# senikm/trpx

Hardware: AMD Instinct MI355X
Metric: frames/s (Terse encode + Prolix decode round trip, 512x512 uint16 stack, bit-exact vs CPU ref) (higher is better)
Workload: dtype u16

## Files before the change

trpx_amd/csrc/encode_fused.hip:

```cpp
#include <stddef.h>
#include <utility>
#include "codec_common.hpp"
#include "launchers.hpp"
#include "profile.hpp"
#include <stdlib.h>
#include <mutex>
#include <vector>

namespace trpx {

#ifndef TRPX_FUSED_SUB32
#define TRPX_FUSED_SUB32 5
#endif
#ifndef TRPX_FUSED_SUB16
#define TRPX_FUSED_SUB16 4
#endif
template <typename T> constexpr int sub_tiles() { return sizeof(T) <= 2 ? TRPX_FUSED_SUB16 : TRPX_FUSED_SUB32; }
#ifndef TRPX_FUSED_OCC16
#define TRPX_FUSED_OCC16 8
#endif
#ifndef TRPX_FUSED_OCC32
#define TRPX_FUSED_OCC32 4
#endif
template <typename T> constexpr int fused_occupancy() { return sizeof(T) == 1 ? 8 : (sizeof(T) == 2 ? TRPX_FUSED_OCC16 : TRPX_FUSED_OCC32); }
[[maybe_unused]] constexpr uint64_t kWaitTicks = 25u * 1000u * 1000u;
struct SpinGuard {
    uint64_t t0 = 0;
    uint32_t spins = 0;
    __device__ __forceinline__ bool expired() {
#ifdef TRPX_FORCE_TIMEOUT
        return true;
#else
        if ((++spins & 63u) != 0u) return false;
        const uint64_t now = __builtin_amdgcn_s_memrealtime();
        if (t0 == 0) { t0 = now; return false; }
        return now - t0 > kWaitTicks;
#endif
    }
};

#ifdef TRPX_DIAGNOSTICS
#define TRPX_DIAG(a) ((a).debug)
#else
#define TRPX_DIAG(a) 0u
#endif

constexpr uint64_t kStInvalid = 0, kStAgg = 1, kStPrefix = 2;
constexpr uint32_t kGridY = 32768;
constexpr int kWmaxShift = 56;
constexpr uint64_t kBndHead = 1ull << 55;
constexpr uint64_t kHeadFlag = 1ull << 63, kTailFlag = 1ull << 62;
__device__ __forceinline__ uint64_t make_desc(uint64_t st, uint64_t v) { return (st << 62) | (v & ((1ull << 62) - 1)); }
__device__ __forceinline__ uint64_t desc_status(uint64_t d) { return d >> 62; }
__device__ __forceinline__ uint64_t desc_value(uint64_t d) { return d & ((1ull << 62) - 1); }

__device__ __forceinline__ uint64_t ld_desc(const uint64_t* p) {
    return __hip_atomic_load(p, __ATOMIC_RELAXED, __HIP_MEMORY_SCOPE_AGENT);
}
__device__ __forceinline__ void st_desc(uint64_t* p, uint64_t v) {
    __hip_atomic_store(p, v, __ATOMIC_RELAXED, __HIP_MEMORY_SCOPE_AGENT);
}

__device__ __forceinline__ uint64_t wave_sum64(uint64_t v) {
    const uint32_t l0 = (uint32_t)v & 0x1FFFFFu, l1 = (uint32_t)(v >> 21) & 0x1FFFFFu, l2 = (uint32_t)(v >> 42);
    const uint32_t s0 = (uint32_t)__builtin_amdgcn_readlane((int)wave_inclusive_scan(l0), 63);
    const uint32_t s1 = (uint32_t)__builtin_amdgcn_readlane((int)wave_inclusive_scan(l1), 63);
    const uint32_t s2 = (uint32_t)__builtin_amdgcn_readlane((int)wave_inclusive_scan(l2), 63);
    return (uint64_t)s0 + ((uint64_t)s1 << 21) + ((uint64_t)s2 << 42);
}

__device__ bool lookback(const uint64_t* __restrict__ desc, int64_t idx, int64_t lo, uint64_t* result) {
    const int lane = lane_id();
    uint64_t acc = 0;
    int64_t pos = idx - 1;
    while (pos >= lo) {
        const int64_t my = pos - lane;
        const bool in = my >= lo;
        uint64_t g = in ? 0ull : make_desc(kStPrefix, 0);
        uint32_t first_p = 64;
        SpinGuard guard;
        uint64_t need = ~0ull;
        for (;;) {
            if (desc_status(g) == kStInvalid && ((need >> lane) & 1ull)) g = ld_desc(desc + my);
            const uint64_t pmask = __ballot(desc_status(g) == kStPrefix);
            const uint64_t imask = __ballot(desc_status(g) == kStInvalid);
            first_p = pmask ? (uint32_t)__builtin_ctzll(pmask) : 64u;
            need = first_p >= 63u ? ~0ull : ((2ull << first_p) - 1ull);
            if ((imask & need) == 0) break;
            if (guard.expired()) return false;
            __builtin_amdgcn_s_sleep(2);
        }
        acc += wave_sum64((uint32_t)lane <= first_p ? desc_value(g) : 0ull);
        if (first_p < 64u) break;
        pos -= 64;
    }
    *result = acc;
    return true;
}

constexpr int kAccShift = 40;
#ifndef TRPX_FUSED_ACC_LINES
#define TRPX_FUSED_ACC_LINES 2
#endif
constexpr uint32_t kAccLines = TRPX_FUSED_ACC_LINES;
__host__ __device__ inline uint32_t fused_acc_lines(uint32_t tiles_per_frame) {
    const uint32_t k = (tiles_per_frame + 31u) / 32u;
    return k < 1u ? 1u : (k > kAccLines ? kAccLines : k);
}
constexpr uint64_t kPrefFlag = 1ull << 63;
__device__ bool lookback_frames(const uint64_t* __restrict__ acc_w, const uint64_t* __restrict__ pref_w, int64_t frame,
                                uint64_t tiles_per_frame, uint64_t* result, uint64_t stride, uint32_t n_acc) {
    const int lane = lane_id();
    uint64_t acc = 0;
    int64_t pos = frame - 1;
    while (pos >= 0) {
        const int64_t my = pos - lane;
        const bool in = my >= 0;
        uint64_t p = in ? 0ull : kPrefFlag, c = 0;
        uint32_t first_p = 64;
        SpinGuard guard;
        uint64_t need = ~0ull;
        bool complete = false;
        for (;;) {
            if (in && !(p & kPrefFlag) && !complete && ((need >> lane) & 1ull)) {
                p = ld_desc(pref_w + my * stride);
                c = ld_desc(acc_w + my * stride);
                for (uint32_t k = 1; k < n_acc; ++k) c += ld_desc(acc_w + my * stride + 16u * k);
                complete = (c >> kAccShift) == tiles_per_frame;
            }
            const uint64_t pmask = __ballot((p & kPrefFlag) != 0);
            const uint64_t cmask = __ballot(complete);
            first_p = pmask ? (uint32_t)__builtin_ctzll(pmask) : 64u;
            need = first_p >= 64u ? ~0ull : ((1ull << first_p) - 1ull);
            if ((~cmask & need) == 0) break;
            if (guard.expired()) return false;
            __builtin_amdgcn_s_sleep(2);
        }
        const uint64_t mine = (uint32_t)lane < first_p ? 1 + (c & ((1ull << kAccShift) - 1)) / 8
                                                       : ((uint32_t)lane == first_p ? p & ~kPrefFlag : 0ull);
        acc += wave_sum64(mine);
        if (first_p < 64u) break;
        pos -= 64;
    }
    *result = acc;
    return true;
}

template <typename T> struct Raw {
    static constexpr int bits = PixelTraits<T>::bits;
    static constexpr int per = 32 / bits;
    static constexpr int dw = kBlock / per;
};

template <typename T>
__device__ __forceinline__ uint32_t raw_field(const uint32_t (&raw)[Raw<T>::dw], int k) {
    constexpr int per = Raw<T>::per, bits = Raw<T>::bits;
    const uint32_t x = raw[k / per] >> ((k % per) * bits);
    return bits == 32 ? x : x & ((1u << (bits & 31)) - 1u);
}

template <typename T> struct QuadVec;
template <> struct QuadVec<uint8_t>  { typedef uint32_t type; };
template <> struct QuadVec<int8_t>   { typedef uint32_t type; };
template <> struct QuadVec<uint16_t> { typedef uint32_t type __attribute__((ext_vector_type(2))); };
template <> struct QuadVec<int16_t>  { typedef uint32_t type __attribute__((ext_vector_type(2))); };
template <> struct QuadVec<uint32_t> { typedef uint32_t type __attribute__((ext_vector_type(4))); };
template <> struct QuadVec<int32_t>  { typedef uint32_t type __attribute__((ext_vector_type(4))); };

template <typename T>
__device__ __forceinline__ void load_raw_nt(const T* __restrict__ p, uint32_t (&raw)[Raw<T>::dw]) {
    if constexpr (sizeof(T) == 2) {
        typedef uint32_t u4 __attribute__((ext_vector_type(4)));
        typedef uint32_t u2 __attribute__((ext_vector_type(2)));
        u4 lo; u2 hi;
        __builtin_memcpy(&lo, p, 16);
        __builtin_memcpy(&hi, reinterpret_cast<const char*>(p) + 16, 8);
        raw[0] = lo.x; raw[1] = lo.y; raw[2] = lo.z; raw[3] = lo.w; raw[4] = hi.x; raw[5] = hi.y;
        return;
    } else if constexpr (sizeof(T) == 1) {
        typedef uint32_t u3 __attribute__((ext_vector_type(3)));
        u3 x;
        __builtin_memcpy(&x, p, 12);
        raw[0] = x.x; raw[1] = x.y; raw[2] = x.z;
        return;
    }
    using V = typename QuadVec<T>::type;
    constexpr int q = Raw<T>::dw / 3;
    const V* src = reinterpret_cast<const V*>(p);
    union U { V vec; uint32_t x[q]; };
    U a, b, c;
    a.vec = src[0];
    b.vec = src[1];
    c.vec = src[2];
#pragma unroll
    for (int i = 0; i < q; ++i) { raw[i] = a.x[i]; raw[q + i] = b.x[i]; raw[2 * q + i] = c.x[i]; }
}
template <typename T>
__device__ __forceinline__ void load_raw_mis2(const T* __restrict__ p, uint32_t (&raw)[Raw<T>::dw]) {
    static_assert(sizeof(T) == 2, "16-bit pixels");
    typedef uint32_t u4 __attribute__((ext_vector_type(4)));
    typedef uint32_t u2 __attribute__((ext_vector_type(2)));
    const char* q = reinterpret_cast<const char*>(p) - 2;
    u4 lo; u2 hi; uint16_t last;
    __builtin_memcpy(&lo, q, 16);
    __builtin_memcpy(&hi, q + 16, 8);
    __builtin_memcpy(&last, q + 24, 2);
    raw[0] = __builtin_amdgcn_alignbit(lo.y, lo.x, 16); raw[1] = __builtin_amdgcn_alignbit(lo.z, lo.y, 16);
    raw[2] = __builtin_amdgcn_alignbit(lo.w, lo.z, 16); raw[3] = __builtin_amdgcn_alignbit(hi.x, lo.w, 16);
    raw[4] = __builtin_amdgcn_alignbit(hi.y, hi.x, 16); raw[5] = __builtin_amdgcn_alignbit((uint32_t)last, hi.y, 16);
}
template <typename T>
__device__ __forceinline__ void load_raw_partial(const T* __restrict__ p, int nb, uint32_t (&raw)[Raw<T>::dw]) {
    using UT = typename PixelTraits<T>::U;
#pragma unroll
    for (int i = 0; i < Raw<T>::dw; ++i) raw[i] = 0;
#pragma unroll
    for (int k = 0; k < kBlock; ++k)
        if (k < nb) raw[k / Raw<T>::per] |= (uint32_t)(UT)p[k] << ((k % Raw<T>::per) * Raw<T>::bits);
}

template <typename T>
__device__ __forceinline__ uint32_t raw_width(const uint32_t (&raw)[Raw<T>::dw]) {
    constexpr int bits = Raw<T>::bits;
    uint32_t m = 0;
    if (!PixelTraits<T>::is_signed) {
#pragma unroll
        for (int i = 0; i < Raw<T>::dw; ++i) m |= raw[i];
        if (bits == 16) m = (m | (m >> 16)) & 0xFFFFu;
        if (bits == 8) { m |= m >> 16; m = (m | (m >> 8)) & 0xFFu; }
    } else if (bits == 32) {
#pragma unroll
        for (int i = 0; i < Raw<T>::dw; ++i) {
            const uint32_t u = raw[i];
            m |= (int32_t)u < 0 ? 0u - u : u;
        }
    } else if (bits == 16) {
        typedef short s2 __attribute__((ext_vector_type(2)));
        typedef unsigned short us2 __attribute__((ext_vector_type(2)));
        uint32_t acc = 0;
#pragma unroll
        for (int i = 0; i < Raw<T>::dw; ++i) {
            union { uint32_t u; s2 v; us2 w; } x, n, y;
            x.u = raw[i];
            n.w = (us2)(0) - x.w;
            y.v = __builtin_elementwise_max(x.v, n.v);
            acc |= y.u;
        }
        m = (acc | (acc >> 16)) & 0xFFFFu;
    } else {
#pragma unroll
        for (int k = 0; k < kBlock; ++k) {
            const int32_t x = (int32_t)(int8_t)(raw[k / 4] >> ((k % 4) * 8));
            m |= (uint32_t)(x < 0 ? -x : x);
        }
    }
    return width_from_or<T>(m);
}

template <int ND>
__device__ __forceinline__ void lds_or_string(uint32_t* __restrict__ stage, uint32_t pos, uint32_t hv_top,
                                              const uint32_t* __restrict__ p) {
    const uint32_t d = (pos + 31u) >> 5, rs = (0u - pos) & 31u;
    const uint32_t xm = __builtin_amdgcn_alignbit(hv_top, 0u, rs);
    if (xm) atomicOr(&stage[d - 1], xm);
    if constexpr (ND == 0) {
        const uint32_t x0 = __builtin_amdgcn_alignbit(0u, hv_top, rs);
        if (x0) atomicOr(&stage[d], x0);
    } else {
        atomicOr(&stage[d], __builtin_amdgcn_alignbit(p[0], hv_top, rs));
#pragma unroll
        for (int j = 1; j < ND; ++j) {
            const uint32_t x = __builtin_amdgcn_alignbit(p[j], p[j - 1], rs);
            if (j >= ND - 1) atomicOr(&stage[d + j], x);
            else stage[d + j] = x;
        }
        const uint32_t x = __builtin_amdgcn_alignbit(0u, p[ND - 1], rs);
        if (x) atomicOr(&stage[d + ND], x);
    }
}

template <typename T, int W>
__device__ __forceinline__ void pack_payload_w(uint32_t* __restrict__ stage, uint32_t pos, uint32_t hv_top,
                                               const uint32_t (&raw)[Raw<T>::dw]) {
    constexpr int NB = kBlock * W;
    constexpr int ND = (NB + 31) / 32;
    constexpr int per = Raw<T>::per, bits = Raw<T>::bits;
    constexpr uint32_t MASK = W >= 32 ? 0xFFFFFFFFu : ((1u << (W & 31)) - 1u);
    uint32_t p[ND ? ND : 1];
#pragma unroll
    for (int j = 0; j < ND; ++j) p[j] = 0;
    if constexpr (W == 0) {
    } else if constexpr (bits == 16 && W < 16) {
        typedef unsigned short us2 __attribute__((ext_vector_type(2)));
        constexpr int L = (15 - W) / (2 * W) + 1;
        constexpr uint32_t kPairMask = MASK | (MASK << 16);
#pragma unroll
        for (int c = 0; c * L < kBlock / 2; ++c) {
            uint32_t acc = 0;
            int n_pairs = 0;
#pragma unroll
            for (int i = 0; i < L; ++i) {
                const int j = c * L + i;
                if (j < kBlock / 2) {
                    union { uint32_t u; us2 v; } x, k;
                    x.u = PixelTraits<T>::is_signed ? raw[j] & kPairMask : raw[j];
                    k.u = (1u << (2 * W * i)) | (1u << (2 * W * i + W + 16));
                    acc = __builtin_amdgcn_udot2(x.v, k.v, acc, false);
                    ++n_pairs;
                }
            }
            const int bit = 2 * W * L * c, nbits = 2 * W * n_pairs;
            p[bit >> 5] |= acc << (bit & 31);
            if ((bit & 31) + nbits > 32) p[(bit >> 5) + 1] |= acc >> (32 - (bit & 31));
        }
    } else if constexpr (bits == 16) {
#pragma unroll
        for (int j = 0; j < kBlock / 2; ++j) p[j] = raw[j];
    } else {
#pragma unroll
        for (int k = 0; k < kBlock; ++k) {
            const uint32_t u = (raw[k / per] >> ((k % per) * bits)) & MASK;
            const int bit = k * W;
            p[bit >> 5] |= u << (bit & 31);
            if ((bit & 31) + W > 32) p[(bit >> 5) + 1] |= u >> (32 - (bit & 31));
        }
    }
    lds_or_string<ND>(stage, pos, hv_top, p);
}

template <typename T, int LO, int HI>
struct PackDispatch {
    static __device__ __forceinline__ void run(uint32_t* stage, uint32_t pos, uint32_t hv_top, uint32_t w0,
                                               const uint32_t (&raw)[Raw<T>::dw]) {
        if constexpr (LO == HI) pack_payload_w<T, LO>(stage, pos, hv_top, raw);
        else {
            constexpr int MID = (LO + HI) / 2;
            if (w0 <= (uint32_t)MID) PackDispatch<T, LO, MID>::run(stage, pos, hv_top, w0, raw);
            else PackDispatch<T, MID + 1, HI>::run(stage, pos, hv_top, w0, raw);
        }
    }
};

template <typename T>
__device__ __forceinline__ void pack_payload_generic(uint32_t* __restrict__ stage, uint32_t pos, uint32_t w, int nb,
                                                     const uint32_t (&raw)[Raw<T>::dw]) {
    const uint32_t mask = w >= 32u ? 0xFFFFFFFFu : ((1u << w) - 1u);
#pragma unroll
    for (int k = 0; k < kBlock; ++k) {
        if (k < nb) {
            const uint64_t x = (uint64_t)(raw_field<T>(raw, k) & mask) << (pos & 31u);
            if ((uint32_t)x) atomicOr(&stage[pos >> 5], (uint32_t)x);
            if ((uint32_t)(x >> 32)) atomicOr(&stage[(pos >> 5) + 1], (uint32_t)(x >> 32));
            pos += w;
        }
    }
}

template <typename T> constexpr int fused_phase_rounds() { return (sub_tiles<T>() + 1) / 2; }
template <typename T>
constexpr int fused_stage_dwords() { return fused_phase_rounds<T>() * ((kThreads * max_block_bits<T>() + 31) / 32) + 12; }

struct FusedArgs {
    FrameGeom g;
    uint32_t n_frames;
    uint32_t tiles_per_frame;
    uint64_t out_capacity;
    uint64_t* tile_desc;
    uint64_t* tail_desc;
    uint64_t* bnd_pos;
    uint64_t* frame_acc;
    uint64_t* frame_pref;
    uint64_t* frame_base;
    uint32_t acc_stride;
    uint32_t n_acc;
    uint64_t* ws_tag;
    uint64_t expect_tag;
    uint64_t* frame_offsets;
    uint32_t* out32;
    uint32_t* status;
    uint8_t* idx_widths;
    uint64_t* idx_group_off;
    uint32_t debug;
    uint64_t* stamps;
};

typedef const char __attribute__((address_space(4)))* karg_ptr;
#define TRPX_KARG(kb, field) (*reinterpret_cast<const decltype(FusedArgs::field) __attribute__((address_space(4)))*>((kb) + 8 + offsetof(FusedArgs, field)))

template <typename T, bool MIS2>
__device__ __forceinline__ void encode_fused_body(const T* __restrict__ pixels, const FusedArgs& a) {
    constexpr int kSub = sub_tiles<T>();
    constexpr int kFusedTileBlocks = kSub * kThreads;
    constexpr int kStage = fused_stage_dwords<T>();
    constexpr int kStage4 = (kStage + 1 + 3) / 4;
    __shared__ __attribute__((aligned(16))) uint32_t s_stage_pad[4 * kStage4];
    uint32_t* const s_stage = s_stage_pad + 1;
    __shared__ uint32_t s_hdr[40];
    __shared__ uint32_t s_wtot[kSub * 4];
    __shared__ uint32_t s_wfl[kSub * 4];
    __shared__ uint64_t s_excl_bits;
    __shared__ uint64_t s_base_bytes;
    __shared__ uint32_t s_abort;
    __shared__ uint32_t s_carry;
    __shared__ uint32_t s_halo;

    const uint32_t tid = threadIdx.x;
#define TRPX_STAMP(slot) do { if ((TRPX_DIAG(a) & 4u) && threadIdx.x == 0) a.stamps[((uint64_t)(blockIdx.z * kGridY + blockIdx.y) * gridDim.x + blockIdx.x) * 8 + (slot)] = __builtin_amdgcn_s_memrealtime(); } while (0)
    TRPX_STAMP(0);
    const int lane = lane_id(), wave = wave_id();
    const FrameGeom g = a.g;
    const uint32_t t = blockIdx.x;
    const uint32_t frame = blockIdx.z * kGridY + blockIdx.y;
    const uint32_t n_frames = a.n_frames, tpf = a.tiles_per_frame;
    asm volatile("" :: "s"(g.n_values), "s"(g.n_blocks), "s"(n_frames), "s"(tpf), "s"(pixels));
    if (frame >= n_frames) return;
    const uint64_t tile = (uint64_t)frame * tpf + t;
    const bool last_tile_of_frame = t + 1 == tpf;
    if (tile == 0 && tid == 0) {
        karg_ptr kb0 = (karg_ptr)__builtin_amdgcn_kernarg_segment_ptr();
        uint64_t* const st64 = reinterpret_cast<uint64_t*>(TRPX_KARG(kb0, status));
#pragma unroll
        for (int i = 0; i < 4; ++i) st_desc(st64 + i, 0ull);
        const uint64_t want = TRPX_KARG(kb0, expect_tag);
        if (want != 0ull && ld_desc(TRPX_KARG(kb0, ws_tag)) != want) atomicMax(&TRPX_KARG(kb0, status)[0], 7u);
        asm volatile("s_waitcnt vmcnt(0)" ::: "memory");
    }
    const T* fp = pixels + (uint64_t)frame * g.n_values;
    const uint32_t b0 = t * kFusedTileBlocks;

    uint32_t v[kSub][Raw<T>::dw];
    uint32_t w[kSub], up[kSub], len[kSub], inc[kSub];
    int nb[kSub];
    const bool has_full = g.n_values >= (uint64_t)kBlock;
    const uint64_t max_first = has_full ? g.n_values - kBlock : 0;
    uint32_t h[Raw<T>::dw];
    [[maybe_unused]] const bool mis2 = MIS2 && ((uintptr_t)fp & 2u) != 0u && frame != 0u;
    if (has_full) {
        bool loaded = false;
        if constexpr (MIS2 && sizeof(T) == 2) {
            if (mis2) {
#pragma unroll
                for (int r = 0; r < kSub; ++r) {
                    const uint64_t first = (uint64_t)(b0 + r * kThreads + tid) * kBlock;
                    load_raw_mis2<T>(fp + (first < max_first ? first : max_first), v[r]);
                }
                loaded = true;
            }
        }
        if (!loaded) {
#pragma unroll
            for (int r = 0; r < kSub; ++r) {
                const uint64_t first = (uint64_t)(b0 + r * kThreads + tid) * kBlock;
                load_raw_nt<T>(fp + (first < max_first ? first : max_first), v[r]);
            }
        }
        if (wave == 0) load_raw_nt<T>(fp + (uint64_t)(b0 ? b0 - 1 : 0) * kBlock, h);
        else {
#pragma unroll
            for (int i = 0; i < Raw<T>::dw; ++i) h[i] = 0u;
        }
    } else {
#pragma unroll
        for (int r = 0; r < kSub; ++r)
#pragma unroll
            for (int i = 0; i < Raw<T>::dw; ++i) v[r][i] = 0u;
#pragma unroll
        for (int i = 0; i < Raw<T>::dw; ++i) h[i] = 0u;
    }
    const uint32_t nb_tail = (uint32_t)(g.n_values - (uint64_t)(g.n_blocks - 1) * kBlock);
#pragma unroll
    for (int r = 0; r < kSub; ++r) {
        const uint32_t b1 = b0 + r * kThreads + tid + 1u;
        nb[r] = b1 < g.n_blocks ? kBlock : (b1 == g.n_blocks ? (int)nb_tail : 0);
    }
    if (tid == 0) s_abort = 0;
    if (tid <= 32u) s_hdr[tid] = header_val(tid, tid + 1u) << (32u - header_len(tid, tid + 1u));
    {
        typedef uint32_t u4 __attribute__((ext_vector_type(4)));
        u4* z = reinterpret_cast<u4*>(s_stage_pad);
#pragma unroll
        for (int i = 0; i < (kStage4 + kThreads - 1) / kThreads; ++i)
            if (i * kThreads + (int)tid < kStage4) z[i * kThreads + tid] = (u4)(0u);
    }
    uint32_t pv[Raw<T>::dw];
#pragma unroll
    for (int i = 0; i < Raw<T>::dw; ++i) pv[i] = 0u;
    if (last_tile_of_frame && g.n_values % kBlock) {
        const uint32_t bp = g.n_blocks - 1;
        if (bp >= b0 && (bp - b0) % kThreads == tid) load_raw_partial<T>(fp + (uint64_t)bp * kBlock, (int)(g.n_values % kBlock), pv);
    }
    TRPX_STAMP(7);
    uint32_t w_part = 0u;
    if (last_tile_of_frame && g.n_values % kBlock) w_part = raw_width<T>(pv);
    if (wave == 0) {
        const uint32_t hw0 = b0 > 0 ? raw_width<T>(h) : 0u;
        if (lane == 0) s_halo = hw0;
    }
    uint32_t wmax = 0;
    uint32_t hlr[kSub];
#pragma unroll
    for (int r = 0; r < kSub; ++r) {
        w[r] = nb[r] == kBlock ? raw_width<T>(v[r]) : (nb[r] ? w_part : 0u);
        wmax = w[r] > wmax ? w[r] : wmax;
        if (a.idx_widths && nb[r]) a.idx_widths[(uint64_t)frame * g.n_blocks + b0 + r * kThreads + tid] = (uint8_t)w[r];
        up[r] = (uint32_t)__builtin_amdgcn_update_dpp(0, (int)w[r], 0x138, 0xf, 0xf, false);
        hlr[r] = header_len(w[r], up[r]);
        len[r] = nb[r] ? (lane ? hlr[r] : 0u) + (uint32_t)nb[r] * w[r] : 0u;
    }
    static_assert(kWave * max_block_bits<T>() < 65536, "packed scan needs 16-bit wave totals");
#pragma unroll
    for (int r = 0; r + 1 < kSub; r += 2) {
        const uint32_t two = wave_inclusive_scan(len[r] | (len[r + 1] << 16));
        inc[r] = two & 0xFFFFu;
        inc[r + 1] = two >> 16;
    }
    if (kSub & 1) inc[kSub - 1] = wave_inclusive_scan(len[kSub - 1]);
    const uint32_t wmax_wave = wave_max(wmax);
#pragma unroll
    for (int r = 0; r < kSub; ++r) {
        const uint32_t w_first = (uint32_t)__builtin_amdgcn_readfirstlane((int)w[r]);
        const uint32_t v_first = (uint32_t)__builtin_amdgcn_readfirstlane(nb[r]);
        if (lane == 63) {
            s_wtot[r * 4 + wave] = inc[r];
            s_wfl[r * 4 + wave] = w_first | (w[r] << 8) | ((v_first ? 1u : 0u) << 16) | (r == 0 ? wmax_wave << 24 : 0u);
        }
    }
    TRPX_STAMP(5);
    __syncthreads();
    TRPX_STAMP(1);

    const uint32_t tile_halo = s_halo;
    uint32_t rb[kSub + 1];
    uint32_t off[kSub];
    uint32_t meta[kSub];
    {
        uint32_t tot = 0, h0 = 0, wprev = 0;
        if (lane < kSub * 4) {
            const uint32_t wfl = s_wfl[lane];
            wprev = lane == 0 ? tile_halo : (s_wfl[lane - 1] >> 8) & 0xFFu;
            h0 = (wfl >> 16) & 1u ? header_len(wfl & 0xFFu, wprev) : 0u;
            tot = s_wtot[lane] + h0;
        }
        const uint32_t incl = wave_inclusive_scan(tot);
        const uint32_t excl = incl - tot;
        const uint32_t hw = h0 | (wprev << 8);
        const int swave = __builtin_amdgcn_readfirstlane(wave);
#pragma unroll
        for (int r = 0; r < kSub; ++r) {
            rb[r] = (uint32_t)__builtin_amdgcn_readlane((int)excl, r * 4);
            const uint32_t pb = (uint32_t)__builtin_amdgcn_readlane((int)excl, r * 4 + swave);
            const uint32_t ph = (uint32_t)__builtin_amdgcn_readlane((int)hw, r * 4 + swave);
            off[r] = pb + (lane ? (ph & 0xFFu) : 0u) + inc[r] - len[r];
            const uint32_t wp_r = lane ? up[r] : ph >> 8;
            const uint32_t hl_r = lane ? hlr[r] : (ph & 0xFFu);
            meta[r] = w[r] | (wp_r << 8) | (hl_r << 16) | (nb[r] == kBlock ? 1u << 24 : 0u) | (nb[r] ? 1u << 25 : 0u);
        }
        rb[kSub] = (uint32_t)__builtin_amdgcn_readlane((int)incl, kSub * 4 - 1);
    }
    const uint32_t tile_total = rb[kSub];

    if (tid == 0 && !(TRPX_DIAG(a) & 1u)) {
        st_desc(a.tile_desc + tile, make_desc(t == 0 ? kStPrefix : kStAgg, tile_total));
        __hip_atomic_fetch_add(a.frame_acc + (uint64_t)frame * a.acc_stride + 16u * (t % a.n_acc), (1ull << kAccShift) | tile_total, __ATOMIC_RELAXED, __HIP_MEMORY_SCOPE_AGENT);
    }
    constexpr int kPhaseRounds = fused_phase_rounds<T>();
    constexpr uint32_t kCapBits = (uint32_t)kPhaseRounds * kThreads * max_block_bits<T>();
    const bool two_phase = tile_total > kCapBits;
    uint64_t p0 = 0, p_end = 0;
    uint64_t img_p0 = 0;
    uint32_t bias = 0;
    bool writable = false;
#ifndef TRPX_ABLATE
#define TRPX_ABLATE 0
#endif
#define TRPX_WSTAMP(slot) do { if ((TRPX_DIAG(a) & 8u) && lane == 0 && tile < 4096) a.stamps[tile * 32 + wave * 8 + (slot)] = __builtin_amdgcn_s_memrealtime(); } while (0)
    auto pack_round = [&](auto rc) {
        constexpr int r = decltype(rc)::value;
        const uint32_t pos = off[r] - bias;
        const uint32_t mr = meta[r];
        const uint32_t hl = (mr >> 16) & 0xFFu;
        const uint32_t wr = mr & 0xFFu;
        const uint32_t hv_top = wr == ((mr >> 8) & 0xFFu) ? 0x80000000u : s_hdr[wr];
        const bool full = (mr >> 24) & 1u;
        if (((mr >> 25) & 1u) && !full && !(TRPX_ABLATE & 2)) {
            const uint64_t hx = (uint64_t)(hv_top >> (32u - hl)) << (pos & 31u);
            atomicOr(&s_stage[pos >> 5], (uint32_t)hx);
            if ((uint32_t)(hx >> 32)) atomicOr(&s_stage[(pos >> 5) + 1], (uint32_t)(hx >> 32));
            if (wr) pack_payload_generic<T>(s_stage, pos + hl, wr, (int)nb_tail, pv);
        }
        uint64_t todo = (TRPX_ABLATE & 1) ? 0ull : __ballot(full);
        while (todo) {
            const int l0 = __builtin_ctzll(todo);
            const uint32_t w0 = (uint32_t)__builtin_amdgcn_readlane((int)wr, l0);
            const bool mine = full && wr == w0;
            uint32_t wd = w0;
            asm volatile("" : "+s"(wd));
#pragma unroll
            for (int i = 0; i < Raw<T>::dw; ++i) asm volatile("" : "+v"(v[r][i]));
            if (mine) PackDispatch<T, 0, PixelTraits<T>::bits>::run(s_stage_pad, pos + hl, hv_top, wd, v[r]);
            todo &= ~__ballot(mine);
        }
        TRPX_WSTAMP(1 + r);
    };
    auto look_back = [&]() {
        if (wave == 0) {
            uint64_t excl = 0;
            bool ok = true;
            if (TRPX_DIAG(a) & 1u) excl = (uint64_t)t * 40000u;
            else if (t != 0) {
                ok = lookback(a.tile_desc, (int64_t)tile, (int64_t)(tile - t), &excl);
                if (ok && lane == 0) st_desc(a.tile_desc + tile, make_desc(kStPrefix, excl + tile_total));
            }
            if (lane == 0) { s_excl_bits = excl; if (!ok) s_abort = 1; }
            TRPX_STAMP(2);
        } else if (wave == 1) {
            uint64_t base = 0;
            bool ok = true;
            if (TRPX_DIAG(a) & 1u) base = (uint64_t)frame * 120000u;
            else if (t == 0) {
                ok = lookback_frames(a.frame_acc, a.frame_pref, (int64_t)frame, a.tiles_per_frame, &base, a.acc_stride, a.n_acc);
                if (ok && lane == 0) st_desc(a.frame_base + (uint64_t)frame * 16, kPrefFlag | base);
            } else {
                uint64_t vb = 0;
                SpinGuard guard;
                for (;;) {
                    vb = ld_desc(a.frame_base + (uint64_t)frame * 16);
                    if (vb & kPrefFlag) break;
                    if (guard.expired()) { ok = false; break; }
                    __builtin_amdgcn_s_sleep(2);
                }
                base = vb & ~kPrefFlag;
            }
            if (lane == 0) { s_base_bytes = base; if (!ok) s_abort = 1; }
        }
    };
    auto place_tile = [&]() -> bool {
        karg_ptr kb = (karg_ptr)__builtin_amdgcn_kernarg_segment_ptr();
        asm volatile("" : "+s"(kb));
        const bool aborted = s_abort != 0;
        const uint64_t excl_bits = s_excl_bits, base_bytes = s_base_bytes;
        const uint64_t frame_size = 1 + (excl_bits + tile_total) / 8;
        if (last_tile_of_frame && tid == 0 && !aborted) {
            st_desc(TRPX_KARG(kb, frame_pref) + (uint64_t)frame * TRPX_KARG(kb, acc_stride), kPrefFlag | (base_bytes + frame_size));
            TRPX_KARG(kb, frame_offsets)[frame + 1] = base_bytes + frame_size;
            if (frame == 0) TRPX_KARG(kb, frame_offsets)[0] = 0;
            if (frame + 1 == TRPX_KARG(kb, n_frames) && align_up(base_bytes + frame_size, 4) > TRPX_KARG(kb, out_capacity))
                atomicMax(&TRPX_KARG(kb, status)[0], 3u);
        }
        if (aborted) {
            if (tid == 0) atomicMax(&TRPX_KARG(kb, status)[0], 7u);
            return false;
        }
        if (TRPX_KARG(kb, idx_group_off) && tid < (uint32_t)kSub && b0 + tid * kThreads < g.n_blocks) {
            uint32_t rbv = 0;
#pragma unroll
            for (int r = 0; r < kSub; ++r) rbv = tid == (uint32_t)r ? rb[r] : rbv;
            TRPX_KARG(kb, idx_group_off)[(uint64_t)frame * g.n_tiles + (uint64_t)t * kSub + tid] = excl_bits + rbv;
        }
        p0 = 8 * base_bytes + excl_bits;
        p_end = last_tile_of_frame ? 8 * (base_bytes + frame_size) : p0 + tile_total;
        writable = align_up((p_end + 7) / 8, 4) <= TRPX_KARG(kb, out_capacity);
        img_p0 = p0;
        return true;
    };
    auto flush = [&](bool first, bool carry_out, uint64_t q_end) {
        karg_ptr kb = (karg_ptr)__builtin_amdgcn_kernarg_segment_ptr();
        asm volatile("" : "+s"(kb));
        uint32_t* const out32 = TRPX_KARG(kb, out32);
        uint64_t* const tail_desc = TRPX_KARG(kb, tail_desc);
        const uint32_t s0 = (uint32_t)(img_p0 & 31), sh = (32u - s0) & 31u;
        const bool head_pending = s0 != 0;
        const uint64_t d_first = img_p0 >> 5, d_last = q_end >> 5;
        const int32_t k_first = head_pending ? -1 : 0;
        const uint32_t n_out = (uint32_t)(d_last - d_first);
        const bool completed_first = d_last > d_first;
        const bool is_last_tile = tile + 1 == (uint64_t)TRPX_KARG(kb, n_frames) * TRPX_KARG(kb, tiles_per_frame);
        if (tid == 0) {
            const int32_t kt = k_first + (int32_t)n_out;
            const uint32_t tail_bits = (q_end & 31) ? __builtin_amdgcn_alignbit(s_stage[kt + 1], s_stage[kt], sh) : 0u;
            if (head_pending) {
                const uint32_t head_bits = __builtin_amdgcn_alignbit(s_stage[0], 0u, sh);
                __hip_atomic_fetch_or(tail_desc + tile, kHeadFlag | head_bits, __ATOMIC_RELAXED, __HIP_MEMORY_SCOPE_AGENT);
            }
            if (first) {
                uint32_t wm = 0;
#pragma unroll
                for (int i = 0; i < 4; ++i) wm = (s_wfl[i] >> 24) > wm ? (s_wfl[i] >> 24) : wm;
                TRPX_KARG(kb, bnd_pos)[tile] = (head_pending ? d_first | kBndHead : 0ull) | ((uint64_t)wm << kWmaxShift);
            }
            if (carry_out) s_carry = tail_bits;
            else if ((q_end & 31) != 0 && (completed_first || !head_pending)) {
                if (is_last_tile) { if (writable) __builtin_nontemporal_store(tail_bits, out32 + d_last); }
                else __hip_atomic_fetch_or(tail_desc + tile + 1, kTailFlag | tail_bits, __ATOMIC_RELAXED, __HIP_MEMORY_SCOPE_AGENT);
            }
        }
        if (!(TRPX_ABLATE & 4) && writable) {
            typedef uint32_t u4 __attribute__((ext_vector_type(4)));
            uint32_t al = (0u - ((uint32_t)((uintptr_t)out32 >> 2) + (uint32_t)d_first)) & 3u;
            if (head_pending && al == 0) al = 4;
            al = al < n_out ? al : n_out;
            const uint32_t n4 = (n_out - al) >> 2, rest0 = al + 4 * n4;
            if (tid < al + (n_out - rest0)) {
                const uint32_t j = tid < al ? tid : rest0 + (tid - al);
                if (!(j == 0 && head_pending)) {
                    const int32_t k = k_first + (int32_t)j;
                    __builtin_nontemporal_store(__builtin_amdgcn_alignbit(s_stage[k + 1], s_stage[k], sh), out32 + d_first + j);
                }
            }
            const uint32_t kk0 = (uint32_t)(k_first + 1) + al;
            const uint32_t m = kk0 & 3u;
            const u4* pad4 = reinterpret_cast<const u4*>(s_stage_pad) + (kk0 >> 2);
            u4* dst = reinterpret_cast<u4*>(out32 + d_first + al);
#ifdef TRPX_ENC_PLAIN_STORES
#define TRPX_STREAM_STORE(v, p) (*(p) = (v))
#else
#define TRPX_STREAM_STORE(v, p) __builtin_nontemporal_store(v, p)
#endif
#define TRPX_FLUSH_GROUPS(M)                                                                                   \
            for (uint32_t gq = tid; gq < n4; gq += kThreads) {                                                 \
                const u4 A = pad4[gq], B = pad4[gq + 1];                                                       \
                const uint32_t e[8] = {A.x, A.y, A.z, A.w, B.x, B.y, B.z, B.w};                                \
                u4 x;                                                                                          \
                x.x = __builtin_amdgcn_alignbit(e[M + 1], e[M + 0], sh);                                       \
                x.y = __builtin_amdgcn_alignbit(e[M + 2], e[M + 1], sh);                                       \
                x.z = __builtin_amdgcn_alignbit(e[M + 3], e[M + 2], sh);                                       \
                x.w = __builtin_amdgcn_alignbit(e[M + 4], e[M + 3], sh);                                       \
                TRPX_STREAM_STORE(x, dst + gq);                                                                \
            }
            if (m == 0) { TRPX_FLUSH_GROUPS(0) } else if (m == 1) { TRPX_FLUSH_GROUPS(1) }
            else if (m == 2) { TRPX_FLUSH_GROUPS(2) } else { TRPX_FLUSH_GROUPS(3) }
#undef TRPX_FLUSH_GROUPS
        }
    };

    TRPX_WSTAMP(0);
    [&]<int... R>(std::integer_sequence<int, R...>) { (pack_round(std::integral_constant<int, R>{}), ...); }(std::make_integer_sequence<int, kPhaseRounds>{});
    if (two_phase) {
        look_back();
        __syncthreads();
        if (!place_tile()) return;
        flush(true, true, p0 + rb[kPhaseRounds]);
        const uint64_t d_last = (p0 + rb[kPhaseRounds]) >> 5;
        __syncthreads();
        {
            typedef uint32_t u4 __attribute__((ext_vector_type(4)));
            u4* z = reinterpret_cast<u4*>(s_stage_pad);
            for (int i = (int)tid; i < kStage4; i += kThreads) z[i] = (u4)(0u);
        }
        __syncthreads();
        if (tid == 0 && s_carry) atomicOr(&s_stage[0], s_carry);
        img_p0 = 32 * d_last;
        bias = (uint32_t)(img_p0 - p0);
    }
    [&]<int... R>(std::integer_sequence<int, R...>) { (pack_round(std::integral_constant<int, kPhaseRounds + R>{}), ...); }(std::make_integer_sequence<int, kSub - kPhaseRounds>{});
    if (!two_phase) look_back();
    __syncthreads();
    TRPX_STAMP(3);
    if (!two_phase && !place_tile()) return;
    flush(!two_phase, false, p_end);
    TRPX_STAMP(4);
    if ((TRPX_DIAG(a) & 4u) && tid == 0) { uint32_t xcc; asm volatile("s_getreg_b32 %0, hwreg(HW_REG_XCC_ID)" : "=s"(xcc)); a.stamps[tile * 8 + 6] = xcc; }
}

template <typename T>
__global__ __launch_bounds__(kThreads, fused_occupancy<T>()) void k_encode_fused(const T* __restrict__ pixels, FusedArgs a) {
    encode_fused_body<T, false>(pixels, a);
}
template <typename T>
__global__ __launch_bounds__(kThreads, fused_occupancy<T>() - 1) void k_encode_fused_mis2(const T* __restrict__ pixels, FusedArgs a) {
    encode_fused_body<T, true>(pixels, a);
}

__global__ __launch_bounds__(kThreads) void k_stitch(uint64_t* __restrict__ tile_desc, uint64_t* __restrict__ xw, const uint64_t* __restrict__ pos,
                                                     uint64_t n_tiles, uint64_t* __restrict__ frame_words, uint64_t n_frame_words,
                                                     uint64_t* __restrict__ ws_tag, uint64_t tag, uint32_t* __restrict__ out32,
                                                     uint64_t out_capacity, uint32_t* __restrict__ status) {
    __shared__ uint32_t s_max[4];
    const uint64_t b = (uint64_t)blockIdx.x * kThreads + threadIdx.x;
    constexpr uint64_t kPosMask = kBndHead - 1;
    const bool in = b < n_tiles;
    const uint32_t st0 = __hip_atomic_load(&status[0], __ATOMIC_RELAXED, __HIP_MEMORY_SCOPE_AGENT);
    const uint64_t pw = in ? pos[b] : 0ull;
    const uint64_t pb = in && b > 0 ? pos[b - 1] : 0ull;
    const uint64_t xb = in ? xw[b] : 0ull;
    const bool failed = st0 != 0u;
    const uint32_t wm = wave_max(failed ? 0u : (uint32_t)(pw >> kWmaxShift));
    if (lane_id() == 0) s_max[wave_id()] = wm;
    __syncthreads();
    if (threadIdx.x == 0) {
        uint32_t m = s_max[0];
        for (int i = 1; i < 4; ++i) m = s_max[i] > m ? s_max[i] : m;
        if (m) atomicMax(&status[1], m);
    }
    for (uint64_t i = b; i < n_frame_words; i += (uint64_t)gridDim.x * kThreads) frame_words[i] = 0ull;
    if (b == 0 && ws_tag) ws_tag[0] = tag;
    if (b >= n_tiles) return;
    tile_desc[b] = 0ull;
    if (failed || b == 0) { xw[b] = 0ull; return; }
    if (!(pw & kBndHead)) { xw[b] = 0ull; return; }
    const uint64_t d = pw & kPosMask;
    if (b > 1 && (pb & kBndHead) && (pb & kPosMask) == d) return;
    uint32_t acc = (uint32_t)xb;
    xw[b] = 0ull;
    for (uint64_t k = b + 1; k < n_tiles; ++k) {
        const uint64_t pk = pos[k];
        if (!((pk & kBndHead) && (pk & kPosMask) == d)) break;
        acc |= (uint32_t)xw[k];
        xw[k] = 0ull;
    }
    if (4 * d + 4 <= out_capacity) out32[d] = acc;
}

template <typename T>
static uint32_t fused_tiles_per_frame(const FrameGeom& g) {
    constexpr uint32_t tb = sub_tiles<T>() * kThreads;
    return (g.n_blocks + tb - 1) / tb;
}

size_t fused_workspace_bytes(const FrameGeom& g, size_t n_frames) {
    const size_t tpf = ((size_t)g.n_blocks + 2 * kThreads - 1) / (2 * kThreads);
    return align_up(8 * (3 * n_frames * tpf + 16 * ((size_t)kAccLines + 1) * n_frames + 1), 256) + 64 * n_frames * tpf;
}

namespace {
struct CleanSig {
    uint32_t elem, tiles_per_frame, n_frames, n_blocks;
    bool operator==(const CleanSig& o) const { return elem == o.elem && tiles_per_frame == o.tiles_per_frame && n_frames == o.n_frames && n_blocks == o.n_blocks; }
};
struct CleanWs { int device; const void* ptr; CleanSig sig; uint64_t tag; };
std::mutex g_clean_mu;
std::vector<CleanWs> g_clean;
uint64_t g_next_tag = 0x5452505800000001ull;
}
void fused_ws_forget(const void* lo, size_t bytes, const void* keep) {
    std::lock_guard<std::mutex> lk(g_clean_mu);
    const char* a = static_cast<const char*>(lo);
    for (size_t i = 0; i < g_clean.size();) {
        const char* p = static_cast<const char*>(g_clean[i].ptr);
        if (p != keep && (!lo || (p >= a && p < a + bytes))) { g_clean[i] = g_clean.back(); g_clean.pop_back(); } else ++i;
    }
}

template <typename T>
static hipError_t launch_fused_t(const EncodeArgs& e, void* ws, hipStream_t st) {
    FusedArgs a;
    a.g = e.geom;
    a.n_frames = e.n_frames;
    a.tiles_per_frame = fused_tiles_per_frame<T>(e.geom);
    a.out_capacity = e.out_capacity;
    const size_t tiles = (size_t)e.n_frames * a.tiles_per_frame;
    a.tile_desc = static_cast<uint64_t*>(ws);
    a.tail_desc = a.tile_desc + tiles;
    a.bnd_pos = a.tail_desc + tiles;
    a.n_acc = fused_acc_lines(a.tiles_per_frame);
    a.acc_stride = 16u * a.n_acc;
    a.frame_acc = a.bnd_pos + tiles;
    a.frame_pref = a.frame_acc + 1;
    a.frame_base = a.frame_acc + (size_t)a.acc_stride * e.n_frames;
    a.frame_offsets = e.frame_offsets;
    a.out32 = reinterpret_cast<uint32_t*>(e.out);
    a.status = e.status;
    a.idx_widths = e.idx_widths;
    a.idx_group_off = e.idx_group_off;
    const size_t frame_words = 16 * ((size_t)a.n_acc + 1) * e.n_frames;
    uint64_t* const frame_words_base = a.frame_acc;
    a.ws_tag = frame_words_base + frame_words;
    a.stamps = reinterpret_cast<uint64_t*>(static_cast<char*>(ws) + align_up(8 * (3 * tiles + frame_words + 1), 256));
#ifdef TRPX_DIAGNOSTICS
    a.debug = getenv("TRPX_FUSED_DEBUG") ? (uint32_t)atoi(getenv("TRPX_FUSED_DEBUG")) : 0u;
#else
    a.debug = 0u;
#endif
    hipStreamCaptureStatus cap = hipStreamCaptureStatusNone;
    if (hipStreamIsCapturing(st, &cap) != hipSuccess) { (void)hipGetLastError(); cap = hipStreamCaptureStatusActive; }
    const bool capturing = cap != hipStreamCaptureStatusNone;
    int device = -1;
    (void)hipGetDevice(&device);
    const CleanSig sig{(uint32_t)sizeof(T), a.tiles_per_frame, e.n_frames, e.geom.n_blocks};
    uint64_t expect = 0, tag = 0;
    if (!capturing) {
        std::lock_guard<std::mutex> lk(g_clean_mu);
        tag = g_next_tag++;
        for (size_t i = 0; i < g_clean.size(); ++i)
            if (g_clean[i].device == device && g_clean[i].ptr == ws) {
                if (g_clean[i].sig == sig) expect = g_clean[i].tag;
                g_clean[i] = g_clean.back(); g_clean.pop_back();
                break;
            }
    }
    a.expect_tag = expect;
    Profiler& prof = profiler();
    prof.begin();
    prof.mark(st);
    if (expect == 0)
        hipLaunchKernelGGL(k_zero_words<0>, dim3(256), dim3(kThreads), 0, st, static_cast<uint64_t*>(ws),
                           (uint64_t)(3 * tiles + frame_words + (capturing ? 0 : 1)), reinterpret_cast<uint64_t*>(e.status), (uint64_t)4);
    prof.mark(st);
    const dim3 grid(a.tiles_per_frame, e.n_frames < kGridY ? e.n_frames : kGridY, (e.n_frames + kGridY - 1) / kGridY);
    bool mis2 = false;
    if constexpr (sizeof(T) == 2) mis2 = (((uintptr_t)e.pixels & 2u) != 0u || (e.geom.n_values & 1u) != 0u) && e.n_frames > 1u;
    if constexpr (sizeof(T) == 2) {
        if (mis2) hipLaunchKernelGGL((k_encode_fused_mis2<T>), grid, dim3(kThreads), 0, st, static_cast<const T*>(e.pixels), a);
    }
    if (!mis2) hipLaunchKernelGGL((k_encode_fused<T>), grid, dim3(kThreads), 0, st, static_cast<const T*>(e.pixels), a);
    prof.mark(st);
    hipLaunchKernelGGL(k_stitch, dim3((uint32_t)((tiles + kThreads - 1) / kThreads)), dim3(kThreads), 0, st,
                       a.tile_desc, a.tail_desc, static_cast<const uint64_t*>(a.bnd_pos), (uint64_t)tiles, frame_words_base, (uint64_t)frame_words,
                       capturing ? static_cast<uint64_t*>(nullptr) : a.ws_tag, tag, a.out32, (uint64_t)e.out_capacity, a.status);
    prof.mark(st);
    const hipError_t err = hipGetLastError();
    if (err == hipSuccess && !capturing) {
        std::lock_guard<std::mutex> lk(g_clean_mu);
        if (g_clean.size() >= 64) g_clean.erase(g_clean.begin());
        g_clean.push_back(CleanWs{device, ws, sig, tag});
    }
    return err;
}

hipError_t launch_encode_fused(int dtype, const EncodeArgs& e, void* ws, hipStream_t st) {
    return for_pixel_type(dtype, [&]<class T>() { return launch_fused_t<T>(e, ws, st); });
}

}
```

Measured before the change: 3.723 million.

## Specialize edge-block handling to last tile and retune u16 sub-tiles/occupancy

Moves all partial/empty-block bookkeeping (nb arrays, tail header handling) into branches taken only on the last tile of each frame, so interior tiles compute widths, lengths and payload positions with a simpler path. Per-round metadata is cut from off/meta packs to a payload position plus a byte offset into a header table, with a new entry for the 'same width' header. Load addresses use 32-bit offsets from a tile base pointer. For u16 it raises sub-tiles per thread from 4 to 5 and lowers occupancy targets to 7. This trades register pressure and occupancy for more work per block and fewer per-block instructions.

```diff
diff --git a/trpx_amd/csrc/encode_fused.hip b/trpx_amd/csrc/encode_fused.hip
--- a/trpx_amd/csrc/encode_fused.hip
+++ b/trpx_amd/csrc/encode_fused.hip
@@ -13,11 +13,17 @@
 #define TRPX_FUSED_SUB32 5
 #endif
 #ifndef TRPX_FUSED_SUB16
-#define TRPX_FUSED_SUB16 4
-#endif
-template <typename T> constexpr int sub_tiles() { return sizeof(T) <= 2 ? TRPX_FUSED_SUB16 : TRPX_FUSED_SUB32; }
+#define TRPX_FUSED_SUB16 5
+#endif
+#ifndef TRPX_FUSED_SUB8
+#define TRPX_FUSED_SUB8 4
+#endif
+template <typename T> constexpr int sub_tiles() { return sizeof(T) == 1 ? TRPX_FUSED_SUB8 : (sizeof(T) == 2 ? TRPX_FUSED_SUB16 : TRPX_FUSED_SUB32); }
 #ifndef TRPX_FUSED_OCC16
-#define TRPX_FUSED_OCC16 8
+#define TRPX_FUSED_OCC16 7
+#endif
+#ifndef TRPX_FUSED_OCC16_MIS2
+#define TRPX_FUSED_OCC16_MIS2 7
 #endif
 #ifndef TRPX_FUSED_OCC32
 #define TRPX_FUSED_OCC32 4
@@ -430,29 +436,38 @@
 
     uint32_t v[kSub][Raw<T>::dw];
     uint32_t w[kSub], up[kSub], len[kSub], inc[kSub];
-    int nb[kSub];
     const bool has_full = g.n_values >= (uint64_t)kBlock;
     const uint64_t max_first = has_full ? g.n_values - kBlock : 0;
+    const uint32_t nb_tail = (uint32_t)(g.n_values - (uint64_t)(g.n_blocks - 1) * kBlock);
+    auto edge_nb = [&](int r) -> uint32_t {
+        const uint32_t b1 = b0 + r * kThreads + tid + 1u;
+        return b1 < g.n_blocks ? (uint32_t)kBlock : (b1 == g.n_blocks ? nb_tail : 0u);
+    };
     uint32_t h[Raw<T>::dw];
     [[maybe_unused]] const bool mis2 = MIS2 && ((uintptr_t)fp & 2u) != 0u && frame != 0u;
     if (has_full) {
+        uint64_t tile_first = (uint64_t)b0 * kBlock;
+        uint32_t max_off = 0xFFFFFFFFu;
+        if (last_tile_of_frame) {
+            if (max_first >= tile_first) max_off = (uint32_t)(max_first - tile_first) * (uint32_t)sizeof(T);
+            else { tile_first = max_first; max_off = 0u; }
+        }
+        const char* const tp = reinterpret_cast<const char*>(fp + tile_first);
+        auto block_ptr = [&](int r) -> const T* {
+            const uint32_t ofs = (uint32_t)(r * kThreads + tid) * (uint32_t)(kBlock * sizeof(T));
+            return reinterpret_cast<const T*>(tp + (ofs < max_off ? ofs : max_off));
+        };
         bool loaded = false;
         if constexpr (MIS2 && sizeof(T) == 2) {
             if (mis2) {
 #pragma unroll
-                for (int r = 0; r < kSub; ++r) {
-                    const uint64_t first = (uint64_t)(b0 + r * kThreads + tid) * kBlock;
-                    load_raw_mis2<T>(fp + (first < max_first ? first : max_first), v[r]);
-                }
+                for (int r = 0; r < kSub; ++r) load_raw_mis2<T>(block_ptr(r), v[r]);
                 loaded = true;
             }
         }
         if (!loaded) {
 #pragma unroll
-            for (int r = 0; r < kSub; ++r) {
-                const uint64_t first = (uint64_t)(b0 + r * kThreads + tid) * kBlock;
-                load_raw_nt<T>(fp + (first < max_first ? first : max_first), v[r]);
-            }
+            for (int r = 0; r < kSub; ++r) load_raw_nt<T>(block_ptr(r), v[r]);
         }
         if (wave == 0) load_raw_nt<T>(fp + (uint64_t)(b0 ? b0 - 1 : 0) * kBlock, h);
         else {
@@ -467,20 +482,16 @@
 #pragma unroll
         for (int i = 0; i < Raw<T>::dw; ++i) h[i] = 0u;
     }
-    const uint32_t nb_tail = (uint32_t)(g.n_values - (uint64_t)(g.n_blocks - 1) * kBlock);
-#pragma unroll
-    for (int r = 0; r < kSub; ++r) {
-        const uint32_t b1 = b0 + r * kThreads + tid + 1u;
-        nb[r] = b1 < g.n_blocks ? kBlock : (b1 == g.n_blocks ? (int)nb_tail : 0);
-    }
     if (tid == 0) s_abort = 0;
-    if (tid <= 32u) s_hdr[tid] = header_val(tid, tid + 1u) << (32u - header_len(tid, tid + 1u));
+    if (tid <= 33u) s_hdr[tid] = tid == 33u ? 0x80000000u : header_val(tid, tid + 1u) << (32u - header_len(tid, tid + 1u));
     {
         typedef uint32_t u4 __attribute__((ext_vector_type(4)));
-        u4* z = reinterpret_cast<u4*>(s_stage_pad);
+        u4 zero = (u4)(0u);
+        uint32_t zo = tid * 16u;
+        asm volatile("" : "+v"(zero), "+v"(zo));
 #pragma unroll
         for (int i = 0; i < (kStage4 + kThreads - 1) / kThreads; ++i)
-            if (i * kThreads + (int)tid < kStage4) z[i * kThreads + tid] = (u4)(0u);
+            if (i * kThreads + (int)tid < kStage4) *reinterpret_cast<u4*>(reinterpret_cast<char*>(s_stage_pad) + zo + i * kThreads * 16) = zero;
     }
     uint32_t pv[Raw<T>::dw];
 #pragma unroll
@@ -496,16 +507,39 @@
         const uint32_t hw0 = b0 > 0 ? raw_width<T>(h) : 0u;
         if (lane == 0) s_halo = hw0;
     }
+    constexpr uint32_t kHdrSame = 33u * 4u;
     uint32_t wmax = 0;
-    uint32_t hlr[kSub];
+    uint32_t hk[kSub], q[kSub];
+#pragma unroll
+    for (int r = 0; r < kSub; ++r) w[r] = raw_width<T>(v[r]);
+    if (last_tile_of_frame) {
+#pragma unroll
+        for (int r = 0; r < kSub; ++r) {
+            const uint32_t nb = edge_nb(r);
+            w[r] = nb == (uint32_t)kBlock ? w[r] : (nb ? w_part : 0u);
+        }
+    }
 #pragma unroll
     for (int r = 0; r < kSub; ++r) {
-        w[r] = nb[r] == kBlock ? raw_width<T>(v[r]) : (nb[r] ? w_part : 0u);
         wmax = w[r] > wmax ? w[r] : wmax;
-        if (a.idx_widths && nb[r]) a.idx_widths[(uint64_t)frame * g.n_blocks + b0 + r * kThreads + tid] = (uint8_t)w[r];
         up[r] = (uint32_t)__builtin_amdgcn_update_dpp(0, (int)w[r], 0x138, 0xf, 0xf, false);
-        hlr[r] = header_len(w[r], up[r]);
-        len[r] = nb[r] ? (lane ? hlr[r] : 0u) + (uint32_t)nb[r] * w[r] : 0u;
+        const bool same = w[r] == up[r];
+        const uint32_t hl = same ? 1u : explicit_header_len(w[r]);
+        hk[r] = same ? kHdrSame : w[r] * 4u;
+        len[r] = __umul24(w[r], (uint32_t)kBlock) + (lane ? hl : 0u);
+    }
+    if (last_tile_of_frame) {
+#pragma unroll
+        for (int r = 0; r < kSub; ++r) {
+            const uint32_t nb = edge_nb(r);
+            const uint32_t hl = hk[r] == kHdrSame ? 1u : explicit_header_len(w[r]);
+            len[r] = nb ? (lane ? hl : 0u) + nb * w[r] : 0u;
+        }
+    }
+    if (a.idx_widths) {
+#pragma unroll
+        for (int r = 0; r < kSub; ++r)
+            if (!last_tile_of_frame || edge_nb(r)) a.idx_widths[(uint64_t)frame * g.n_blocks + b0 + r * kThreads + tid] = (uint8_t)w[r];
     }
     static_assert(kWave * max_block_bits<T>() < 65536, "packed scan needs 16-bit wave totals");
 #pragma unroll
@@ -519,11 +553,16 @@
 #pragma unroll
     for (int r = 0; r < kSub; ++r) {
         const uint32_t w_first = (uint32_t)__builtin_amdgcn_readfirstlane((int)w[r]);
-        const uint32_t v_first = (uint32_t)__builtin_amdgcn_readfirstlane(nb[r]);
+        const bool v_first = b0 + r * kThreads + (uint32_t)wave * kWave < g.n_blocks;
         if (lane == 63) {
             s_wtot[r * 4 + wave] = inc[r];
             s_wfl[r * 4 + wave] = w_first | (w[r] << 8) | ((v_first ? 1u : 0u) << 16) | (r == 0 ? wmax_wave << 24 : 0u);
         }
+        q[r] = inc[r] - __umul24(w[r], (uint32_t)kBlock);
+    }
+    if (last_tile_of_frame) {
+#pragma unroll
+        for (int r = 0; r < kSub; ++r) q[r] = inc[r] - edge_nb(r) * w[r];
     }
     TRPX_STAMP(5);
     __syncthreads();
@@ -531,29 +570,26 @@
 
     const uint32_t tile_halo = s_halo;
     uint32_t rb[kSub + 1];
-    uint32_t off[kSub];
-    uint32_t meta[kSub];
+    uint32_t pp[kSub];
     {
-        uint32_t tot = 0, h0 = 0, wprev = 0;
+        uint32_t tot = 0, h0 = 0, hk0 = 0;
         if (lane < kSub * 4) {
             const uint32_t wfl = s_wfl[lane];
-            wprev = lane == 0 ? tile_halo : (s_wfl[lane - 1] >> 8) & 0xFFu;
-            h0 = (wfl >> 16) & 1u ? header_len(wfl & 0xFFu, wprev) : 0u;
+            const uint32_t wprev = lane == 0 ? tile_halo : (s_wfl[lane - 1] >> 8) & 0xFFu;
+            const bool same = (wfl & 0xFFu) == wprev;
+            hk0 = same ? kHdrSame : (wfl & 0xFFu) * 4u;
+            h0 = (wfl >> 16) & 1u ? (same ? 1u : explicit_header_len(wfl & 0xFFu)) : 0u;
             tot = s_wtot[lane] + h0;
         }
         const uint32_t incl = wave_inclusive_scan(tot);
         const uint32_t excl = incl - tot;
-        const uint32_t hw = h0 | (wprev << 8);
+        const uint32_t pay0 = excl + h0;
         const int swave = __builtin_amdgcn_readfirstlane(wave);
 #pragma unroll
         for (int r = 0; r < kSub; ++r) {
             rb[r] = (uint32_t)__builtin_amdgcn_readlane((int)excl, r * 4);
-            const uint32_t pb = (uint32_t)__builtin_amdgcn_readlane((int)excl, r * 4 + swave);
-            const uint32_t ph = (uint32_t)__builtin_amdgcn_readlane((int)hw, r * 4 + swave);
-            off[r] = pb + (lane ? (ph & 0xFFu) : 0u) + inc[r] - len[r];
-            const uint32_t wp_r = lane ? up[r] : ph >> 8;
-            const uint32_t hl_r = lane ? hlr[r] : (ph & 0xFFu);
-            meta[r] = w[r] | (wp_r << 8) | (hl_r << 16) | (nb[r] == kBlock ? 1u << 24 : 0u) | (nb[r] ? 1u << 25 : 0u);
+            pp[r] = (uint32_t)__builtin_amdgcn_readlane((int)pay0, r * 4 + swave) + q[r];
+            hk[r] = lane ? hk[r] : (uint32_t)__builtin_amdgcn_readlane((int)hk0, r * 4 + swave);
         }
         rb[kSub] = (uint32_t)__builtin_amdgcn_readlane((int)incl, kSub * 4 - 1);
     }
@@ -576,19 +612,25 @@
 #define TRPX_WSTAMP(slot) do { if ((TRPX_DIAG(a) & 8u) && lane == 0 && tile < 4096) a.stamps[tile * 32 + wave * 8 + (slot)] = __builtin_amdgcn_s_memrealtime(); } while (0)
     auto pack_round = [&](auto rc) {
         constexpr int r = decltype(rc)::value;
-        const uint32_t pos = off[r] - bias;
-        const uint32_t mr = meta[r];
-        const uint32_t hl = (mr >> 16) & 0xFFu;
-        const uint32_t wr = mr & 0xFFu;
-        const uint32_t hv_top = wr == ((mr >> 8) & 0xFFu) ? 0x80000000u : s_hdr[wr];
-        const bool full = (mr >> 24) & 1u;
-        if (((mr >> 25) & 1u) && !full && !(TRPX_ABLATE & 2)) {
-            const uint64_t hx = (uint64_t)(hv_top >> (32u - hl)) << (pos & 31u);
-            atomicOr(&s_stage[pos >> 5], (uint32_t)hx);
-            if ((uint32_t)(hx >> 32)) atomicOr(&s_stage[(pos >> 5) + 1], (uint32_t)(hx >> 32));
-            if (wr) pack_payload_generic<T>(s_stage, pos + hl, wr, (int)nb_tail, pv);
-        }
-        uint64_t todo = (TRPX_ABLATE & 1) ? 0ull : __ballot(full);
+        const uint32_t pos = pp[r] - bias;
+        const uint32_t wr = w[r];
+        const uint32_t hv_top = *reinterpret_cast<const uint32_t*>(reinterpret_cast<const char*>(s_hdr) + hk[r]);
+        bool full = true;
+        uint64_t todo = __ballot(true);
+        if (last_tile_of_frame) {
+            const uint32_t nb = edge_nb(r);
+            full = nb == (uint32_t)kBlock;
+            if (nb && !full && !(TRPX_ABLATE & 2)) {
+                const uint32_t hl = hk[r] == kHdrSame ? 1u : explicit_header_len(wr);
+                const uint32_t hp = pos - hl;
+                const uint64_t hx = (uint64_t)(hv_top >> (32u - hl)) << (hp & 31u);
+                atomicOr(&s_stage[hp >> 5], (uint32_t)hx);
+                if ((uint32_t)(hx >> 32)) atomicOr(&s_stage[(hp >> 5) + 1], (uint32_t)(hx >> 32));
+                if (wr) pack_payload_generic<T>(s_stage, pos, wr, (int)nb_tail, pv);
+            }
+            todo = __ballot(full);
+        }
+        if (TRPX_ABLATE & 1) todo = 0ull;
         while (todo) {
             const int l0 = __builtin_ctzll(todo);
             const uint32_t w0 = (uint32_t)__builtin_amdgcn_readlane((int)wr, l0);
@@ -597,7 +639,7 @@
             asm volatile("" : "+s"(wd));
 #pragma unroll
             for (int i = 0; i < Raw<T>::dw; ++i) asm volatile("" : "+v"(v[r][i]));
-            if (mine) PackDispatch<T, 0, PixelTraits<T>::bits>::run(s_stage_pad, pos + hl, hv_top, wd, v[r]);
+            if (mine) PackDispatch<T, 0, PixelTraits<T>::bits>::run(s_stage_pad, pos, hv_top, wd, v[r]);
             todo &= ~__ballot(mine);
         }
         TRPX_WSTAMP(1 + r);
@@ -767,7 +809,7 @@
     encode_fused_body<T, false>(pixels, a);
 }
 template <typename T>
-__global__ __launch_bounds__(kThreads, fused_occupancy<T>() - 1) void k_encode_fused_mis2(const T* __restrict__ pixels, FusedArgs a) {
+__global__ __launch_bounds__(kThreads, TRPX_FUSED_OCC16_MIS2) void k_encode_fused_mis2(const T* __restrict__ pixels, FusedArgs a) {
     encode_fused_body<T, true>(pixels, a);
 }
 
```

Result: faster. 3.807 million, median of 6 (+2.3%).
